# AnnaUshnova/tinyrenderder

Measured on AMD Instinct MI355X. Metric: triangles/sec (+ Mpixels/sec) at 4096x4096; achieved HBM GB/s vs peak, higher is better.
Workload: dtype f64

## Files before the change

tinyrenderder_amd/csrc/kernels_bin.hip:

```cpp
#include <hip/hip_runtime.h>
#include "trgl_device.h"
#include "launch.h"

namespace {

__device__ __forceinline__ double dmin3(double a, double b, double c) { double m = a; if (b < m) m = b; if (c < m) m = c; return m; }
__device__ __forceinline__ double dmax3(double a, double b, double c) { double m = a; if (m < b) m = b; if (m < c) m = c; return m; }
__device__ __forceinline__ double dot4(const double* m, const double* v) {
    double sum = 0;
    sum += m[0] * v[0]; sum += m[1] * v[1]; sum += m[2] * v[2]; sum += m[3] * v[3];
    return sum;
}

__device__ __forceinline__ int wave_min_i(int v) {
    for (int o = 32; o; o >>= 1) { int t = __shfl_xor(v, o); v = t < v ? t : v; }
    return v;
}
__device__ __forceinline__ int wave_max_i(int v) {
    for (int o = 32; o; o >>= 1) { int t = __shfl_xor(v, o); v = t > v ? t : v; }
    return v;
}

constexpr int SETUP_THREADS = 256;

__global__ __launch_bounds__(SETUP_THREADS) void k_setup(FrameParams fp, DrawDesc d, DrawDesc* __restrict__ draws_out, int draw_idx,
                                                         TriRec* __restrict__ recs, TriW* __restrict__ recs_w, uint32_t* __restrict__ cnt,
                                                         uint2* __restrict__ tilebox, DevStats* __restrict__ stats,
                                                         uint32_t* __restrict__ blk_sums, uint32_t blk_base) {
    __shared__ __attribute__((aligned(16))) double s_buf[SETUP_THREADS * 16];
    if (blockIdx.x == 0 && threadIdx.x == 0) draws_out[draw_idx] = d;
    const uint32_t b0 = blockIdx.x * SETUP_THREADS;
    const uint32_t nb = min((uint32_t)SETUP_THREADS, d.n - b0);
    const uint32_t tid = threadIdx.x;
    const uint32_t i = b0 + tid;
    const bool in_range = tid < nb;

    const double* src = d.clip + (size_t)b0 * 12;
    if ((reinterpret_cast<uintptr_t>(src) & 15) == 0) {
        const double2* s2 = reinterpret_cast<const double2*>(src);
        double2* l2 = reinterpret_cast<double2*>(s_buf);
        typedef double f64x2 __attribute__((ext_vector_type(2)));
        for (uint32_t k = tid; k < nb * 6; k += SETUP_THREADS)
            *reinterpret_cast<f64x2*>(&l2[k]) = __builtin_nontemporal_load(reinterpret_cast<const f64x2*>(&s2[k]));
    } else {
        for (uint32_t k = tid; k < nb * 12; k += SETUP_THREADS) s_buf[k] = src[k];
    }
    __syncthreads();
    double v[12];
#pragma unroll
    for (int k = 0; k < 12; ++k) v[k] = in_range ? s_buf[tid * 12 + k] : 0.0;
    __syncthreads();

    int bx0 = INT_MAX, by0 = INT_MAX, bx1 = INT_MIN, by1 = INT_MIN;
    uint32_t ntiles = 0;
    bool large = false;
    uint2 tb = make_uint2(0, 0);
    TriRec r;
    {
        uint4* z4 = reinterpret_cast<uint4*>(&r);
#pragma unroll
        for (int k = 0; k < 8; ++k) z4[k] = make_uint4(0, 0, 0, 0);
    }
    if (in_range) {
        bool ok = !(v[3] <= 1e-12 || v[7] <= 1e-12 || v[11] <= 1e-12);
        double ndc[12];
#pragma unroll
        for (int q = 0; q < 3; ++q) {
#pragma unroll
            for (int k = 0; k < 3; ++k) ndc[4 * q + k] = v[4 * q + k] / v[4 * q + 3];
            ndc[4 * q + 3] = __builtin_isfinite(v[4 * q + 3]) ? 1.0 : __builtin_nan("");
        }
        bool zo0 = (ndc[2] < -1.0 || ndc[2] > 1.0), zo1 = (ndc[6] < -1.0 || ndc[6] > 1.0),
             zo2 = (ndc[10] < -1.0 || ndc[10] > 1.0);
        ok = ok && !(zo0 && zo1 && zo2);
#pragma unroll
        for (int k = 0; k < 12; ++k) ok = ok && __builtin_isfinite(ndc[k]);
        double sx[3], sy[3];
#pragma unroll
        for (int q = 0; q < 3; ++q) { sx[q] = dot4(fp.vp, ndc + 4 * q); sy[q] = dot4(fp.vp + 4, ndc + 4 * q); }
        double e1x = sx[1] - sx[0], e1y = sy[1] - sy[0], e2x = sx[2] - sx[0], e2y = sy[2] - sy[0];
        double cross_product = e1x * e2y - e1y * e2x;
        ok = ok && !(cross_product <= 0);
        int min_x_px = max(0, x86_cvttsd2si(floor(dmin3(sx[0], sx[1], sx[2]))));
        int max_x_px = min(fp.W - 1, x86_cvttsd2si(ceil(dmax3(sx[0], sx[1], sx[2]))));
        int min_y_px = max(0, x86_cvttsd2si(floor(dmin3(sy[0], sy[1], sy[2]))));
        int max_y_px = min(fp.H - 1, x86_cvttsd2si(ceil(dmax3(sy[0], sy[1], sy[2]))));
        ok = ok && !(min_x_px > max_x_px || min_y_px > max_y_px);
        if (ok) {
            bx0 = min_x_px; by0 = min_y_px; bx1 = max_x_px; by1 = max_y_px;
            r.ax = sx[0]; r.ay = sy[0];
            r.s0x = sx[2] - sx[0]; r.s0y = sx[1] - sx[0];
            r.s1x = sy[2] - sy[0]; r.s1y = sy[1] - sy[0];
            r.uz = r.s0x * r.s1y - r.s0y * r.s1x;
            {
                const double BIG = 0x1p200, SMALL = 0x1p-250;
                bool ws = r.uz < 0.0 && !(fabs(r.uz) < 1e-12);
#pragma unroll
                for (int q = 0; q < 3; ++q) ws = ws && fabs(sx[q]) < BIG && fabs(sy[q]) < BIG;
                const double dl[4] = { r.s0x, r.s0y, r.s1x, r.s1y };
#pragma unroll
                for (int q = 0; q < 4; ++q) ws = ws && (dl[q] == 0.0 || fabs(dl[q]) >= SMALL);
                {
                    const double S = (fabs(r.s0x) + fabs(r.s0y)) + (fabs(r.s1x) + fabs(r.s1y));
                    const double rx = fmax(fabs(r.ax - ((double)bx0 + 0.5)), fabs(r.ax - ((double)bx1 + 0.5)));
                    const double ry = fmax(fabs(r.ay - ((double)by0 + 0.5)), fabs(r.ay - ((double)by1 + 0.5)));
                    ws = ws && 0x1p-40 * (S * S) * (rx + ry + 17.0 + S) < fabs(r.uz);
                }
                r.ruz = ws ? 1.0 / r.uz : 0.0;
            }
            r.z0 = ndc[2]; r.z1 = ndc[6]; r.z2 = ndc[10];
            r.bx0 = (uint16_t)bx0; r.by0 = (uint16_t)by0; r.bx1 = (uint16_t)bx1; r.by1 = (uint16_t)by1;
            r.color = d.colors ? d.colors[i] : 0xffffffffu;
            r.dl = ((uint32_t)draw_idx << 24) | i | (r.ruz == 0.0 ? TRGL_DL_LITERAL : 0u);
            r.c0 = -__builtin_inf(); r.g1 = 0.0; r.g2 = 0.0;
            if (r.ruz != 0.0) {
                const double zabs = dmax3(fabs(r.z0), fabs(r.z1), fabs(r.z2));
                const double dz1 = r.z1 - r.z0, dz2 = r.z2 - r.z0;
                const double h1 = (r.s1x * dz1 - r.s1y * dz2) * r.ruz, h2 = (r.s0y * dz2 - r.s0x * dz1) * r.ruz;
                const double rx = fmax(fabs(r.ax - ((double)bx0 + 0.5)), fabs(r.ax - ((double)bx1 + 0.5)));
                const double ry = fmax(fabs(r.ay - ((double)by0 + 0.5)), fabs(r.ay - ((double)by1 + 0.5)));
                const double Ssum = (fabs(r.s0x) + fabs(r.s0y)) + (fabs(r.s1x) + fabs(r.s1y));
                const double R = rx + ry + 1.0 + Ssum;
                const double mz = zabs * 0x1p-39 * (R * Ssum * fabs(r.ruz) + 1.0) + 0x1p-600;
                const bool okp = zabs < 0x1p1000 && R * fabs(h1) < 0x1p900 && R * fabs(h2) < 0x1p900 && mz < 0x1p1000;
                if (okp) { r.c0 = r.z0 - mz; r.g1 = h1; r.g2 = h2; }
            }
            if (d.kind != TRGL_SHADER_FLAT) {
                TriW w;
                w.iw0 = (fabs(v[3]) > 1e-12) ? (1.0 / v[3]) : 0.0;
                w.iw1 = (fabs(v[7]) > 1e-12) ? (1.0 / v[7]) : 0.0;
                w.iw2 = (fabs(v[11]) > 1e-12) ? (1.0 / v[11]) : 0.0;
                w.pad = 0.0;
                recs_w[d.first + i] = w;
            }
            int y_lo = max(by0, fp.strip_y0), y_hi = min(by1, fp.strip_y1 - 1);
            if (!(fabs(r.uz) < 1e-12) && y_lo <= y_hi) {
                uint32_t tx0 = bx0 >> TRGL_TILE_LOG2, tx1 = bx1 >> TRGL_TILE_LOG2;
                uint32_t ty0 = y_lo >> TRGL_TILE_LOG2, ty1 = y_hi >> TRGL_TILE_LOG2;
                const uint32_t rows = fp.il_tiles ? (uint32_t)(il_owned_below(fp, (int)ty1 + 1) - il_owned_below(fp, (int)ty0)) : ty1 - ty0 + 1;
                ntiles = (tx1 - tx0 + 1) * rows;
                tb = make_uint2(((uint32_t)bx0 >> TRGL_BLOCK_LOG2) | (((uint32_t)y_lo >> TRGL_BLOCK_LOG2) << 16),
                                ((uint32_t)bx1 >> TRGL_BLOCK_LOG2) | (((uint32_t)y_hi >> TRGL_BLOCK_LOG2) << 16));
                uint32_t zq = 0;
                if (r.c0 > -__builtin_inf()) {
                    const double zv = dmin3(r.c0, __builtin_fma(-r.s0y, r.g1, __builtin_fma(-r.s1y, r.g2, r.c0)),
                                            __builtin_fma(-r.s0x, r.g1, __builtin_fma(-r.s1x, r.g2, r.c0)));
                    const double t = (zv + 1.0) * 64.0 - 0x1p-20;
                    if (t >= 1.0) zq = t >= 127.0 ? 127u : (uint32_t)x86_cvttsd2si(floor(t));
                }
                tb.x |= (zq & 7u) << 13; tb.y |= ((zq >> 3) & 7u) << 13; tb.y |= (zq >> 6) << 29;
                large = bx1 - bx0 >= 64 || y_hi - y_lo >= 64;
            }
        }
        cnt[d.first + i] = ntiles;
        tilebox[d.first + i] = tb;
    }
    const uint32_t lane = tid & 63, wbase = tid & ~63u;
    {
        uint4* l4 = reinterpret_cast<uint4*>(s_buf);
        const uint4* r4 = reinterpret_cast<const uint4*>(&r);
#pragma unroll
        for (int c = 0; c < 8; ++c) l4[tid * 8 + (c ^ (tid & 7))] = r4[c];
        const unsigned long long keep = __ballot(ntiles != 0);
        __builtin_amdgcn_wave_barrier();
        uint4* dst = reinterpret_cast<uint4*>(recs + d.first + b0 + wbase);
#pragma unroll
        for (int it = 0; it < 8; ++it) {
            const uint32_t k = lane + 64u * it, t = k >> 3, c = k & 7;
            if ((keep >> t) & 1ull) {
                typedef uint32_t u32x4 __attribute__((ext_vector_type(4)));
                __builtin_nontemporal_store(*reinterpret_cast<const u32x4*>(&l4[(wbase + t) * 8 + (c ^ (t & 7))]), reinterpret_cast<u32x4*>(&dst[k]));
            }
        }
    }
    {
        uint32_t ws = ntiles;
        for (int o = 32; o; o >>= 1) ws += __shfl_xor(ws, o);
        __syncthreads();
        uint32_t* s_ws = reinterpret_cast<uint32_t*>(s_buf);
        if (lane == 0) s_ws[tid >> 6] = ws;
        __syncthreads();
        if (tid == 0) blk_sums[blk_base + blockIdx.x] = s_ws[0] + s_ws[1] + s_ws[2] + s_ws[3];
    }
    {
        const unsigned long long lit = __ballot(ntiles != 0 && r.ruz == 0.0);
        if (lit && lane == 0) atomicAdd(&stats->literal_tris, (unsigned long long)__popcll(lit));
        const unsigned long long lrg = __ballot(large);
        if (lrg && lane == 0) atomicAdd(&stats->large_tris, (unsigned long long)__popcll(lrg));
    }
    int wx0 = wave_min_i(bx0), wy0 = wave_min_i(by0), wx1 = wave_max_i(bx1), wy1 = wave_max_i(by1);
    if ((threadIdx.x & 63) == 0 && wx0 != INT_MAX) {
        if (wx0 < __builtin_nontemporal_load(&stats->min_x)) atomicMin(&stats->min_x, wx0);
        if (wy0 < __builtin_nontemporal_load(&stats->min_y)) atomicMin(&stats->min_y, wy0);
        if (wx1 > __builtin_nontemporal_load(&stats->max_x)) atomicMax(&stats->max_x, wx1);
        if (wy1 > __builtin_nontemporal_load(&stats->max_y)) atomicMax(&stats->max_y, wy1);
    }
}

constexpr int SCAN_THREADS = 256;

__device__ __forceinline__ uint32_t wave_incl_scan(uint32_t v) {
    int lane = threadIdx.x & 63;
    for (int o = 1; o < 64; o <<= 1) { uint32_t t = __shfl_up(v, o); if (lane >= o) v += t; }
    return v;
}

__device__ __forceinline__ uint32_t block_excl_scan(uint32_t v, uint32_t* smem , uint32_t* total) {
    uint32_t inc = wave_incl_scan(v);
    int w = threadIdx.x >> 6, lane = threadIdx.x & 63;
    __syncthreads();
    if (lane == 63) smem[w] = inc;
    __syncthreads();
    uint32_t base = 0, tot = 0;
#pragma unroll
    for (int k = 0; k < SCAN_THREADS / 64; ++k) { uint32_t s = smem[k]; if (k < w) base += s; tot += s; }
    *total = tot;
    return base + inc - v;
}

constexpr int EXPAND_CHUNK = 16;

constexpr int SPINE_THREADS = 1024;
__global__ __launch_bounds__(SPINE_THREADS) void k_chunk_spine(const uint32_t* __restrict__ blk_sums, uint32_t nblk,
                                                               uint32_t* __restrict__ chunk_off,
                                                               unsigned long long* __restrict__ total64, unsigned long long* __restrict__ host_copy,
                                                               uint4* __restrict__ bounds16, uint32_t n_half16) {
    __shared__ unsigned long long s_wave[SPINE_THREADS / 64];
    for (uint32_t k = threadIdx.x; k < 2 * n_half16; k += SPINE_THREADS) bounds16[k] = k < n_half16 ? make_uint4(~0u, ~0u, ~0u, ~0u) : make_uint4(0, 0, 0, 0);
    const uint32_t nchunks = (nblk + EXPAND_CHUNK - 1) / EXPAND_CHUNK;
    const int lane = threadIdx.x & 63, w = threadIdx.x >> 6;
    unsigned long long running = 0;
    for (uint32_t start = 0; start < nchunks; start += SPINE_THREADS) {
        const uint32_t c = start + threadIdx.x;
        unsigned long long v = 0;
        if (c < nchunks) {
            const uint32_t q0 = c * EXPAND_CHUNK;
            if (q0 + EXPAND_CHUNK <= nblk) {
                const uint4* p4 = reinterpret_cast<const uint4*>(blk_sums + q0);
#pragma unroll
                for (int k = 0; k < EXPAND_CHUNK / 4; ++k) { const uint4 t = p4[k]; v += (unsigned long long)t.x + t.y + t.z + t.w; }
            } else {
                for (uint32_t q = q0; q < nblk; ++q) v += blk_sums[q];
            }
        }
        unsigned long long inc = v;
        for (int o = 1; o < 64; o <<= 1) { const unsigned long long t = __shfl_up(inc, o); if (lane >= o) inc += t; }
        if (lane == 63) s_wave[w] = inc;
        __syncthreads();
        unsigned long long base = 0, tot = 0;
#pragma unroll
        for (int k = 0; k < SPINE_THREADS / 64; ++k) { const unsigned long long t = s_wave[k]; if (k < w) base += t; tot += t; }
        if (c < nchunks) chunk_off[c] = (uint32_t)(running + base + inc - v);
        running += tot;
        __syncthreads();
    }
    if (threadIdx.x == 0) {
        *total64 = running;
        host_copy[0] = running; host_copy[1] = total64[1]; host_copy[2] = total64[2];
        __threadfence_system();
    }
}

constexpr uint32_t EXPAND_STAGE = 3072;
__device__ __forceinline__ uint32_t tile_block_mask(uint32_t tx, uint32_t ty, uint32_t qx0, uint32_t qy0, uint32_t qx1, uint32_t qy1) {
    const uint32_t c0 = qx0 > 4 * tx ? qx0 - 4 * tx : 0u, c1 = qx1 < 4 * tx + 3 ? qx1 - 4 * tx : 3u;
    const uint32_t r0 = qy0 > 4 * ty ? qy0 - 4 * ty : 0u, r1 = qy1 < 4 * ty + 3 ? qy1 - 4 * ty : 3u;
    return (((2u << c1) - (1u << c0)) & 0xfu) * 0x1111u & ((0xffffu >> (12 - 4 * r1)) & (0xffffu << (4 * r0)));
}
template <bool WIDE>
__global__ __launch_bounds__(256) void k_expand(FrameParams fp, uint32_t first, uint32_t n, int tiles_x, const uint32_t* __restrict__ cnt,
                                                const uint32_t* __restrict__ blk_sums, const uint32_t* __restrict__ chunk_off,
                                                uint32_t blk_base, const uint2* __restrict__ tilebox,
                                                uint32_t* __restrict__ keys, uint32_t* __restrict__ vals, uint16_t* __restrict__ bmask,
                                                const unsigned long long* __restrict__ pairs_total, uint32_t cap) {
    __shared__ uint32_t smem[4];
    __shared__ __attribute__((aligned(16))) uint32_t s_k[EXPAND_STAGE + 4];
    __shared__ __attribute__((aligned(16))) uint32_t s_v[EXPAND_STAGE + 4];
    __shared__ __attribute__((aligned(16))) uint16_t s_m[WIDE ? EXPAND_STAGE + 4 : 4];
    if (*pairs_total > cap) return;
    const uint32_t local = blockIdx.x * blockDim.x + threadIdx.x;
    const uint32_t i = first + local;
    const uint32_t blk = blk_base + blockIdx.x;
    uint32_t c = 0; uint2 tb = make_uint2(0, 0);
    if (local < n) { c = cnt[i]; if (c) tb = tilebox[i]; }
    uint32_t base;
    {
        const uint32_t q0 = blk - blk % EXPAND_CHUNK, l = threadIdx.x & 63u;
        uint32_t part = l < blk - q0 ? blk_sums[q0 + l] : 0u;
        for (int o = 8; o; o >>= 1) part += __shfl_xor(part, o);
        base = chunk_off[blk / EXPAND_CHUNK] + (uint32_t)__builtin_amdgcn_readfirstlane((int)part);
    }
    uint32_t tot;
    const uint32_t o = block_excl_scan(c, smem, &tot);
    const bool staged = tot <= EXPAND_STAGE;
    const uint32_t sh = base & 3u;
    uint32_t* const kdst = keys + base; uint32_t* const vdst = vals + base; uint16_t* const mdst = bmask + base;
    auto put = [&](uint32_t j, uint32_t key, uint32_t iz, uint32_t m) {
        const uint32_t word = WIDE ? key : key | (m << 16);
        if (staged) { s_k[sh + j] = word; s_v[sh + j] = iz; if (WIDE) s_m[sh + j] = (uint16_t)m; }
        else { kdst[j] = word; vdst[j] = iz; if (WIDE) mdst[j] = (uint16_t)m; }
    };
    constexpr uint32_t SMALL = 8;
    if (c && c <= SMALL) {
        const uint32_t qx0 = tb.x & 0x1fff, qy0 = (tb.x >> 16) & 0x1fff, qx1 = tb.y & 0x1fff, qy1 = (tb.y >> 16) & 0x1fff;
        const uint32_t iz = i | ((((tb.x >> 13) & 7u) | (((tb.y >> 13) & 7u) << 3) | ((tb.y >> 29) << 6)) << 25);
        const uint32_t tx0 = qx0 >> 2, ty0 = qy0 >> 2, tx1 = qx1 >> 2;
        uint32_t tx = tx0, row = 0;
        uint32_t ty = fp.il_tiles ? (uint32_t)il_nth_owned_from(fp, (int)ty0, 0) : ty0;
        for (uint32_t k = 0; k < c; ++k) {
            put(o + k, ty * tiles_x + tx, iz, tile_block_mask(tx, ty, qx0, qy0, qx1, qy1));
            if (++tx > tx1) { tx = tx0; ++row; ty = fp.il_tiles ? (uint32_t)il_nth_owned_from(fp, (int)ty0, (int)row) : ty0 + row; }
        }
    }
    unsigned long long big = __ballot(c > SMALL);
    int lane = threadIdx.x & 63;
    while (big) {
        int src = __ffsll((long long)big) - 1;
        big &= big - 1;
        uint32_t cc = __shfl(c, src), oo = __shfl(o, src), ii = __shfl(i, src);
        uint32_t bx = __shfl(tb.x, src), by = __shfl(tb.y, src);
        const uint32_t qx0 = bx & 0x1fff, qy0 = (bx >> 16) & 0x1fff, qx1 = by & 0x1fff, qy1 = (by >> 16) & 0x1fff;
        ii |= (((bx >> 13) & 7u) | (((by >> 13) & 7u) << 3) | ((by >> 29) << 6)) << 25;
        uint32_t tx0 = qx0 >> 2, ty0 = qy0 >> 2, tx1 = qx1 >> 2;
        uint32_t wdt = tx1 - tx0 + 1;
        for (uint32_t k = lane; k < cc; k += 64) {
            uint32_t ty = fp.il_tiles ? (uint32_t)il_nth_owned_from(fp, (int)ty0, (int)(k / wdt)) : ty0 + k / wdt, tx = tx0 + k % wdt;
            put(oo + k, ty * tiles_x + tx, ii, tile_block_mask(tx, ty, qx0, qy0, qx1, qy1));
        }
    }
    if (staged) {
        __syncthreads();
        uint32_t* const kq = keys + (base - sh); uint32_t* const vq = vals + (base - sh); uint16_t* const mq = bmask + (base - sh);
        const uint32_t end = sh + tot;
        for (uint32_t q = threadIdx.x; 4 * q < end; q += 256) {
            const uint32_t j0 = 4 * q;
            if (j0 >= sh && j0 + 4 <= end) {
                *reinterpret_cast<uint4*>(kq + j0) = *reinterpret_cast<const uint4*>(s_k + j0);
                *reinterpret_cast<uint4*>(vq + j0) = *reinterpret_cast<const uint4*>(s_v + j0);
                if (WIDE) *reinterpret_cast<uint2*>(mq + j0) = *reinterpret_cast<const uint2*>(s_m + j0);
            } else {
                for (uint32_t j = j0; j < j0 + 4; ++j)
                    if (j >= sh && j < end) { kq[j] = s_k[j]; vq[j] = s_v[j]; if (WIDE) mq[j] = s_m[j]; }
            }
        }
    }
}

constexpr int RADIX_ROUNDS = 16;
constexpr int RADIX_WAVE_CHUNK = RADIX_ROUNDS * 64;
constexpr uint32_t RADIX_BIG_CAP = 4u << 20;
constexpr int RADIX_MAX_BITS = 8;

__global__ __launch_bounds__(256) void k_radix_hist(const uint32_t* __restrict__ keys, const unsigned long long* __restrict__ pairs_total,
                                                    uint32_t cap, int shift, int bits, uint32_t chunk,
                                                    uint32_t nblocks, uint32_t* __restrict__ hist) {
    __shared__ uint32_t s_cnt[1 << RADIX_MAX_BITS];
    const unsigned long long P64 = *pairs_total;
    const uint32_t P = P64 > cap ? 0u : (uint32_t)P64;
    const uint32_t nb = 1u << bits, mask = nb - 1;
    for (uint32_t b = threadIdx.x; b < nb; b += 256) s_cnt[b] = 0;
    __syncthreads();
    const uint64_t beg = (uint64_t)blockIdx.x * chunk;
    uint64_t end = beg + chunk; if (end > P) end = P;
    for (uint64_t p = beg + 4u * threadIdx.x; p < end; p += 1024) {
        const uint4 q = *reinterpret_cast<const uint4*>(keys + p);
        const uint32_t k[4] = { q.x, q.y, q.z, q.w };
#pragma unroll
        for (int j = 0; j < 4; ++j) if (p + j < end) atomicAdd(&s_cnt[(k[j] >> shift) & mask], 1u);
    }
    __syncthreads();
    for (uint32_t b = threadIdx.x; b < nb; b += 256) hist[(size_t)b * nblocks + blockIdx.x] = s_cnt[b];
}

constexpr int ROWSCAN_THREADS = 1024, ROWSCAN_PER = 8;
__global__ __launch_bounds__(ROWSCAN_THREADS) void k_radix_scan_rows(uint32_t* __restrict__ hist, uint32_t nblocks, uint32_t* __restrict__ totals) {
    __shared__ uint32_t s_wave[ROWSCAN_THREADS / 64];
    uint32_t* row = hist + (size_t)blockIdx.x * nblocks;
    const int lane = threadIdx.x & 63, w = threadIdx.x >> 6;
    uint32_t running = 0;
    for (uint32_t start = 0; start < nblocks; start += ROWSCAN_THREADS * ROWSCAN_PER) {
        const uint32_t base = start + threadIdx.x * ROWSCAN_PER;
        uint32_t v[ROWSCAN_PER], sum = 0;
#pragma unroll
        for (int k = 0; k < ROWSCAN_PER; ++k) { v[k] = (base + k < nblocks) ? row[base + k] : 0; sum += v[k]; }
        uint32_t inc = sum;
        for (int o = 1; o < 64; o <<= 1) { const uint32_t t = __shfl_up(inc, o); if (lane >= o) inc += t; }
        if (lane == 63) s_wave[w] = inc;
        __syncthreads();
        uint32_t wbase = 0, tot = 0;
#pragma unroll
        for (int k = 0; k < ROWSCAN_THREADS / 64; ++k) { const uint32_t t = s_wave[k]; if (k < w) wbase += t; tot += t; }
        uint32_t run = running + wbase + inc - sum;
#pragma unroll
        for (int k = 0; k < ROWSCAN_PER; ++k) { if (base + k < nblocks) row[base + k] = run; run += v[k]; }
        running += tot;
        __syncthreads();
    }
    if (threadIdx.x == 0) totals[blockIdx.x] = running;
}

template <int RADIX_WAVES, bool WIDE, bool LAST>
__global__ __launch_bounds__(RADIX_WAVES * 64) void k_radix_scatter(const uint32_t* __restrict__ keys_in, const uint32_t* __restrict__ vals_in,
                                                                 const uint16_t* __restrict__ msk_in,
                                                                 const unsigned long long* __restrict__ pairs_total, uint32_t cap,
                                                                 int shift, int bits, uint32_t nblocks,
                                                                 const uint32_t* __restrict__ base, const uint32_t* __restrict__ totals,
                                                                 uint32_t* __restrict__ keys_out, uint32_t* __restrict__ vals_out,
                                                                 uint16_t* __restrict__ msk_out,
                                                                 uint32_t* __restrict__ tile_start, uint32_t* __restrict__ tile_end) {
    constexpr int RADIX_THREADS = RADIX_WAVES * 64, RADIX_CHUNK = RADIX_WAVES * RADIX_WAVE_CHUNK;
    __shared__ uint32_t s_cnt[RADIX_WAVES][1 << RADIX_MAX_BITS];
    __shared__ uint32_t s_start[1 << RADIX_MAX_BITS];
    __shared__ uint32_t s_gbase[1 << RADIX_MAX_BITS];
    __shared__ uint32_t s_val[RADIX_CHUNK];
    __shared__ uint32_t s_key[RADIX_CHUNK];
    __shared__ uint16_t s_msk[WIDE ? RADIX_CHUNK : 2];
    const int w = threadIdx.x >> 6, lane = threadIdx.x & 63;
    const unsigned long long P64 = *pairs_total;
    const uint32_t P = P64 > cap ? 0u : (uint32_t)P64;
    if ((uint64_t)blockIdx.x * RADIX_CHUNK >= P) return;
    const uint32_t nb = 1u << bits, mask = nb - 1;
    for (uint32_t b = threadIdx.x; b < nb; b += RADIX_THREADS) {
#pragma unroll
        for (int ww = 0; ww < RADIX_WAVES; ++ww) s_cnt[ww][b] = 0;
        s_gbase[b] = base[(size_t)b * nblocks + blockIdx.x];
    }
    if (w == 0) {
        uint32_t tot[4], run = 0;
#pragma unroll
        for (int q = 0; q < 4; ++q) { const uint32_t d = lane * 4 + q; tot[q] = d < nb ? totals[d] : 0; run += tot[q]; }
        uint32_t inc = run;
        for (int o = 1; o < 64; o <<= 1) { const uint32_t t = __shfl_up(inc, o); if (lane >= o) inc += t; }
        uint32_t ex = inc - run;
#pragma unroll
        for (int q = 0; q < 4; ++q) { const uint32_t d = lane * 4 + q; if (d < nb) s_start[d] = ex; ex += tot[q]; }
    }
    __syncthreads();
    for (uint32_t b = threadIdx.x; b < nb; b += RADIX_THREADS) s_gbase[b] += s_start[b];
    __syncthreads();
    const uint64_t cbeg = (uint64_t)blockIdx.x * RADIX_CHUNK;
    uint64_t cend = cbeg + RADIX_CHUNK; if (cend > P) cend = P;
    const uint32_t n_chunk = (uint32_t)(cend - cbeg);
    const uint64_t wbeg = cbeg + (uint64_t)w * RADIX_WAVE_CHUNK;
    const unsigned long long lt = (1ull << lane) - 1ull;

    uint32_t k[RADIX_ROUNDS], v[RADIX_ROUNDS], rk[RADIX_ROUNDS];
    uint16_t mk[WIDE ? RADIX_ROUNDS : 1];
#pragma unroll
    for (int r = 0; r < RADIX_ROUNDS; ++r) {
        const uint64_t p = wbeg + (uint64_t)r * 64 + lane;
        const bool act = p < cend;
        k[r] = act ? keys_in[p] : 0; v[r] = act ? vals_in[p] : 0;
        if (WIDE) mk[WIDE ? r : 0] = act ? msk_in[p] : (uint16_t)0;
    }
#pragma unroll
    for (int r = 0; r < RADIX_ROUNDS; ++r) {
        const bool act = wbeg + (uint64_t)r * 64 + lane < cend;
        const uint32_t dgt = (k[r] >> shift) & mask;
        unsigned long long same = __ballot(act);
        for (int b = 0; b < bits; ++b) {
            const unsigned long long bal = __ballot((dgt >> b) & 1u);
            same &= ((dgt >> b) & 1u) ? bal : ~bal;
        }
        const uint32_t cur = act ? s_cnt[w][dgt] : 0;
        __builtin_amdgcn_wave_barrier();
        const uint32_t r_in = __popcll(same & lt);
        rk[r] = cur + r_in;
        if (act && r_in == 0) s_cnt[w][dgt] = cur + (uint32_t)__popcll(same);
        __builtin_amdgcn_wave_barrier();
    }
    __syncthreads();
    if (w == 0) {
        uint32_t tot[4], run = 0;
#pragma unroll
        for (int q = 0; q < 4; ++q) {
            const uint32_t d = lane * 4 + q;
            uint32_t t = 0;
            if (d < nb) {
#pragma unroll
                for (int ww = 0; ww < RADIX_WAVES; ++ww) t += s_cnt[ww][d];
            }
            tot[q] = t;
            run += tot[q];
        }
        uint32_t inc = run;
        for (int o = 1; o < 64; o <<= 1) { const uint32_t t = __shfl_up(inc, o); if (lane >= o) inc += t; }
        uint32_t ex = inc - run;
#pragma unroll
        for (int q = 0; q < 4; ++q) { const uint32_t d = lane * 4 + q; if (d < nb) s_start[d] = ex; ex += tot[q]; }
    }
    __syncthreads();
    for (uint32_t d = threadIdx.x; d < nb; d += RADIX_THREADS) {
        uint32_t run = s_start[d];
#pragma unroll
        for (int ww = 0; ww < RADIX_WAVES; ++ww) { const uint32_t c = s_cnt[ww][d]; s_cnt[ww][d] = run; run += c; }
    }
    __syncthreads();
#pragma unroll
    for (int r = 0; r < RADIX_ROUNDS; ++r) {
        if (wbeg + (uint64_t)r * 64 + lane < cend) {
            const uint32_t dgt = (k[r] >> shift) & mask;
            const uint32_t lp = s_cnt[w][dgt] + rk[r];
            s_key[lp] = k[r]; s_val[lp] = v[r];
            if (WIDE) s_msk[lp] = mk[WIDE ? r : 0];
        }
    }
    __syncthreads();
    constexpr uint32_t KEY_MASK = WIDE ? 0xffffffffu : 0xffffu;
    for (uint32_t i = threadIdx.x; i < n_chunk; i += RADIX_THREADS) {
        const uint32_t word = s_key[i];
        const uint32_t dgt = (word >> shift) & mask;
        const uint32_t dst = s_gbase[dgt] + (i - s_start[dgt]);
        vals_out[dst] = s_val[i];
        if (!LAST) {
            keys_out[dst] = word;
            if (WIDE) msk_out[dst] = s_msk[i];
        } else {
            msk_out[dst] = WIDE ? s_msk[i] : (uint16_t)(word >> 16);
            const uint32_t key = word & KEY_MASK;
            if (i == 0 || (s_key[i - 1] & KEY_MASK) != key) atomicMin(&tile_start[key], dst);
            if (i + 1 == n_chunk || (s_key[i + 1] & KEY_MASK) != key) atomicMax(&tile_end[key], dst + 1);
        }
    }
}

}

namespace trgl {

uint32_t setup_num_blocks(uint32_t n) { return (n + SETUP_THREADS - 1) / SETUP_THREADS; }

void launch_setup(hipStream_t s, const FrameParams& fp, const DrawDesc& draw, DrawDesc* draws_dev, int draw_idx, uint32_t n,
                  TriRec* recs, TriW* recs_w, uint32_t* cnt, uint2* tilebox, DevStats* stats, uint32_t* blk_sums, uint32_t blk_base) {
    if (!n) return;
    hipLaunchKernelGGL(k_setup, dim3(setup_num_blocks(n)), dim3(SETUP_THREADS), 0, s, fp, draw, draws_dev, draw_idx, recs, recs_w, cnt, tilebox,
                       stats, blk_sums, blk_base);
}

void launch_chunk_spine(hipStream_t s, const uint32_t* blk_sums, uint32_t nblk, uint32_t* chunk_off, unsigned long long* total64, unsigned long long* host_copy,
                        uint32_t* tile_bounds, size_t half_words) {
    hipLaunchKernelGGL(k_chunk_spine, dim3(1), dim3(SPINE_THREADS), 0, s, blk_sums, nblk, chunk_off, total64, host_copy, (uint4*)tile_bounds,
                       (uint32_t)(half_words / 4));
}

void launch_expand(hipStream_t s, const FrameParams& fp, uint32_t first, uint32_t n, int tiles_x, const uint32_t* cnt, const uint32_t* blk_sums,
                   const uint32_t* chunk_off, uint32_t blk_base, const uint2* tilebox, uint32_t* keys, bool wide, uint32_t* vals, uint16_t* bmask,
                   const unsigned long long* pairs_total, uint32_t cap) {
    if (!n) return;
    if (wide)
        hipLaunchKernelGGL(k_expand<true>, dim3(setup_num_blocks(n)), dim3(SETUP_THREADS), 0, s, fp, first, n, tiles_x, cnt, blk_sums, chunk_off,
                           blk_base, tilebox, keys, vals, bmask, pairs_total, cap);
    else
        hipLaunchKernelGGL(k_expand<false>, dim3(setup_num_blocks(n)), dim3(SETUP_THREADS), 0, s, fp, first, n, tiles_x, cnt, blk_sums, chunk_off,
                           blk_base, tilebox, keys, vals, bmask, pairs_total, cap);
}

static uint32_t radix_waves(uint32_t cap) { return cap >= RADIX_BIG_CAP ? 8u : 4u; }
uint32_t radix_num_workers(uint32_t cap) { const uint64_t chunk = radix_waves(cap) * RADIX_WAVE_CHUNK; return (uint32_t)((cap + chunk - 1) / chunk); }

template <int WAVES, bool WIDE, bool LAST>
static void radix_pass_t(hipStream_t s, const RadixPass& ps, const unsigned long long* pairs_total, uint32_t cap, uint32_t* hist, uint32_t* scan_tmp) {
    const uint32_t nblk = radix_num_workers(cap);
    hipLaunchKernelGGL(k_radix_hist, dim3(nblk), dim3(256), 0, s, ps.keys_in, pairs_total, cap, ps.shift, ps.bits, (uint32_t)(WAVES * RADIX_WAVE_CHUNK),
                       nblk, hist);
    hipLaunchKernelGGL(k_radix_scan_rows, dim3(1u << ps.bits), dim3(ROWSCAN_THREADS), 0, s, hist, nblk, scan_tmp);
    hipLaunchKernelGGL((k_radix_scatter<WAVES, WIDE, LAST>), dim3(nblk), dim3(WAVES * 64), 0, s, ps.keys_in, ps.vals_in, ps.msk_in, pairs_total, cap,
                       ps.shift, ps.bits, nblk, hist, scan_tmp, ps.keys_out, ps.vals_out, ps.msk_out, ps.tile_start, ps.tile_end);
}

template <int WAVES>
static void radix_pass_w(hipStream_t s, const RadixPass& ps, bool wide, bool last, const unsigned long long* pairs_total, uint32_t cap,
                         uint32_t* hist, uint32_t* scan_tmp) {
    if (wide) { if (last) radix_pass_t<WAVES, true, true>(s, ps, pairs_total, cap, hist, scan_tmp); else radix_pass_t<WAVES, true, false>(s, ps, pairs_total, cap, hist, scan_tmp); }
    else { if (last) radix_pass_t<WAVES, false, true>(s, ps, pairs_total, cap, hist, scan_tmp); else radix_pass_t<WAVES, false, false>(s, ps, pairs_total, cap, hist, scan_tmp); }
}

void launch_radix_pass(hipStream_t s, const RadixPass& ps, bool wide, bool last, const unsigned long long* pairs_total, uint32_t cap,
                       uint32_t* hist, uint32_t* scan_tmp) {
    if (!cap) return;
    if (radix_waves(cap) == 8) radix_pass_w<8>(s, ps, wide, last, pairs_total, cap, hist, scan_tmp);
    else radix_pass_w<4>(s, ps, wide, last, pairs_total, cap, hist, scan_tmp);
}

}
```

Before: 4.120 billion.

## Hoist global loads ahead of dependent work in expand and radix kernels

In the expand kernel, the per-block prefix loads (blk_sums, chunk_off, tilebox) are issued before the early-exit check so their latency overlaps. The radix histogram is templated on a fixed step count and issues all of its uint4 key loads up front, clamping the tail address, before doing the shared atomics. The scatter kernel issues the bucket-base and totals loads together with the key/value loads and moves its shared init and scan after them. Its output phase is batched into groups of eight so shared reads and address math are done before the global stores. The cost targeted is serialized memory latency, in exchange for more registers per thread and heavier unrolling, which may lower occupancy.

```diff
diff --git a/tinyrenderder_amd/csrc/kernels_bin.hip b/tinyrenderder_amd/csrc/kernels_bin.hip
--- a/tinyrenderder_amd/csrc/kernels_bin.hip
+++ b/tinyrenderder_amd/csrc/kernels_bin.hip
@@ -277,18 +277,19 @@
     __shared__ __attribute__((aligned(16))) uint32_t s_k[EXPAND_STAGE + 4];
     __shared__ __attribute__((aligned(16))) uint32_t s_v[EXPAND_STAGE + 4];
     __shared__ __attribute__((aligned(16))) uint16_t s_m[WIDE ? EXPAND_STAGE + 4 : 4];
-    if (*pairs_total > cap) return;
     const uint32_t local = blockIdx.x * blockDim.x + threadIdx.x;
     const uint32_t i = first + local;
     const uint32_t blk = blk_base + blockIdx.x;
     uint32_t c = 0; uint2 tb = make_uint2(0, 0);
-    if (local < n) { c = cnt[i]; if (c) tb = tilebox[i]; }
+    if (local < n) { c = cnt[i]; tb = tilebox[i]; }
+    const uint32_t q0 = blk - blk % EXPAND_CHUNK, l = threadIdx.x & 63u;
+    uint32_t part = l < blk - q0 ? blk_sums[q0 + l] : 0u;
+    const uint32_t coff = chunk_off[blk / EXPAND_CHUNK];
+    if (*pairs_total > cap) return;
     uint32_t base;
     {
-        const uint32_t q0 = blk - blk % EXPAND_CHUNK, l = threadIdx.x & 63u;
-        uint32_t part = l < blk - q0 ? blk_sums[q0 + l] : 0u;
         for (int o = 8; o; o >>= 1) part += __shfl_xor(part, o);
-        base = chunk_off[blk / EXPAND_CHUNK] + (uint32_t)__builtin_amdgcn_readfirstlane((int)part);
+        base = coff + (uint32_t)__builtin_amdgcn_readfirstlane((int)part);
     }
     uint32_t tot;
     const uint32_t o = block_excl_scan(c, smem, &tot);
@@ -351,9 +352,10 @@
 constexpr uint32_t RADIX_BIG_CAP = 4u << 20;
 constexpr int RADIX_MAX_BITS = 8;
 
+template <int STEPS>
 __global__ __launch_bounds__(256) void k_radix_hist(const uint32_t* __restrict__ keys, const unsigned long long* __restrict__ pairs_total,
-                                                    uint32_t cap, int shift, int bits, uint32_t chunk,
-                                                    uint32_t nblocks, uint32_t* __restrict__ hist) {
+                                                    uint32_t cap, int shift, int bits, uint32_t nblocks, uint32_t* __restrict__ hist) {
+    constexpr uint32_t chunk = STEPS * 1024;
     __shared__ uint32_t s_cnt[1 << RADIX_MAX_BITS];
     const unsigned long long P64 = *pairs_total;
     const uint32_t P = P64 > cap ? 0u : (uint32_t)P64;
@@ -362,9 +364,18 @@
     __syncthreads();
     const uint64_t beg = (uint64_t)blockIdx.x * chunk;
     uint64_t end = beg + chunk; if (end > P) end = P;
-    for (uint64_t p = beg + 4u * threadIdx.x; p < end; p += 1024) {
-        const uint4 q = *reinterpret_cast<const uint4*>(keys + p);
-        const uint32_t k[4] = { q.x, q.y, q.z, q.w };
+    if (beg >= end) { for (uint32_t b = threadIdx.x; b < nb; b += 256) hist[(size_t)b * nblocks + blockIdx.x] = 0; return; }
+    const uint64_t last4 = (end - 1) & ~(uint64_t)3;
+    uint4 q[STEPS];
+#pragma unroll
+    for (int r = 0; r < STEPS; ++r) {
+        const uint64_t p = beg + 4u * threadIdx.x + 1024u * r;
+        q[r] = *reinterpret_cast<const uint4*>(keys + (p < last4 ? p : last4));
+    }
+#pragma unroll
+    for (int r = 0; r < STEPS; ++r) {
+        const uint64_t p = beg + 4u * threadIdx.x + 1024u * r;
+        const uint32_t k[4] = { q[r].x, q[r].y, q[r].z, q[r].w };
 #pragma unroll
         for (int j = 0; j < 4; ++j) if (p + j < end) atomicAdd(&s_cnt[(k[j] >> shift) & mask], 1u);
     }
@@ -409,6 +420,7 @@
                                                                  uint16_t* __restrict__ msk_out,
                                                                  uint32_t* __restrict__ tile_start, uint32_t* __restrict__ tile_end) {
     constexpr int RADIX_THREADS = RADIX_WAVES * 64, RADIX_CHUNK = RADIX_WAVES * RADIX_WAVE_CHUNK;
+    static_assert(RADIX_THREADS >= (1 << RADIX_MAX_BITS), "one thread per digit");
     __shared__ uint32_t s_cnt[RADIX_WAVES][1 << RADIX_MAX_BITS];
     __shared__ uint32_t s_start[1 << RADIX_MAX_BITS];
     __shared__ uint32_t s_gbase[1 << RADIX_MAX_BITS];
@@ -420,30 +432,17 @@
     const uint32_t P = P64 > cap ? 0u : (uint32_t)P64;
     if ((uint64_t)blockIdx.x * RADIX_CHUNK >= P) return;
     const uint32_t nb = 1u << bits, mask = nb - 1;
-    for (uint32_t b = threadIdx.x; b < nb; b += RADIX_THREADS) {
-#pragma unroll
-        for (int ww = 0; ww < RADIX_WAVES; ++ww) s_cnt[ww][b] = 0;
-        s_gbase[b] = base[(size_t)b * nblocks + blockIdx.x];
-    }
-    if (w == 0) {
-        uint32_t tot[4], run = 0;
-#pragma unroll
-        for (int q = 0; q < 4; ++q) { const uint32_t d = lane * 4 + q; tot[q] = d < nb ? totals[d] : 0; run += tot[q]; }
-        uint32_t inc = run;
-        for (int o = 1; o < 64; o <<= 1) { const uint32_t t = __shfl_up(inc, o); if (lane >= o) inc += t; }
-        uint32_t ex = inc - run;
-#pragma unroll
-        for (int q = 0; q < 4; ++q) { const uint32_t d = lane * 4 + q; if (d < nb) s_start[d] = ex; ex += tot[q]; }
-    }
-    __syncthreads();
-    for (uint32_t b = threadIdx.x; b < nb; b += RADIX_THREADS) s_gbase[b] += s_start[b];
-    __syncthreads();
     const uint64_t cbeg = (uint64_t)blockIdx.x * RADIX_CHUNK;
     uint64_t cend = cbeg + RADIX_CHUNK; if (cend > P) cend = P;
     const uint32_t n_chunk = (uint32_t)(cend - cbeg);
     const uint64_t wbeg = cbeg + (uint64_t)w * RADIX_WAVE_CHUNK;
     const unsigned long long lt = (1ull << lane) - 1ull;
 
+    const uint32_t dq = min((uint32_t)threadIdx.x, nb - 1);
+    const uint32_t gcol = base[(size_t)dq * nblocks + blockIdx.x];
+    uint32_t tot[4];
+#pragma unroll
+    for (int q = 0; q < 4; ++q) { const uint32_t d = lane * 4 + q; tot[q] = totals[min(d, nb - 1)]; if (d >= nb) tot[q] = 0; }
     uint32_t k[RADIX_ROUNDS], v[RADIX_ROUNDS], rk[RADIX_ROUNDS];
     uint16_t mk[WIDE ? RADIX_ROUNDS : 1];
 #pragma unroll
@@ -453,6 +452,24 @@
         k[r] = act ? keys_in[p] : 0; v[r] = act ? vals_in[p] : 0;
         if (WIDE) mk[WIDE ? r : 0] = act ? msk_in[p] : (uint16_t)0;
     }
+    if (threadIdx.x < nb) {
+#pragma unroll
+        for (int ww = 0; ww < RADIX_WAVES; ++ww) s_cnt[ww][threadIdx.x] = 0;
+        s_gbase[threadIdx.x] = gcol;
+    }
+    if (w == 0) {
+        uint32_t run = 0;
+#pragma unroll
+        for (int q = 0; q < 4; ++q) run += tot[q];
+        uint32_t inc = run;
+        for (int o = 1; o < 64; o <<= 1) { const uint32_t t = __shfl_up(inc, o); if (lane >= o) inc += t; }
+        uint32_t ex = inc - run;
+#pragma unroll
+        for (int q = 0; q < 4; ++q) { const uint32_t d = lane * 4 + q; if (d < nb) s_start[d] = ex; ex += tot[q]; }
+    }
+    __syncthreads();
+    if (threadIdx.x < nb) s_gbase[threadIdx.x] += s_start[threadIdx.x];
+
 #pragma unroll
     for (int r = 0; r < RADIX_ROUNDS; ++r) {
         const bool act = wbeg + (uint64_t)r * 64 + lane < cend;
@@ -490,8 +507,10 @@
         for (int q = 0; q < 4; ++q) { const uint32_t d = lane * 4 + q; if (d < nb) s_start[d] = ex; ex += tot[q]; }
     }
     __syncthreads();
-    for (uint32_t d = threadIdx.x; d < nb; d += RADIX_THREADS) {
+    if (threadIdx.x < nb) {
+        const uint32_t d = threadIdx.x;
         uint32_t run = s_start[d];
+        s_gbase[d] -= run;
 #pragma unroll
         for (int ww = 0; ww < RADIX_WAVES; ++ww) { const uint32_t c = s_cnt[ww][d]; s_cnt[ww][d] = run; run += c; }
     }
@@ -507,19 +526,39 @@
     }
     __syncthreads();
     constexpr uint32_t KEY_MASK = WIDE ? 0xffffffffu : 0xffffu;
-    for (uint32_t i = threadIdx.x; i < n_chunk; i += RADIX_THREADS) {
-        const uint32_t word = s_key[i];
-        const uint32_t dgt = (word >> shift) & mask;
-        const uint32_t dst = s_gbase[dgt] + (i - s_start[dgt]);
-        vals_out[dst] = s_val[i];
-        if (!LAST) {
-            keys_out[dst] = word;
-            if (WIDE) msk_out[dst] = s_msk[i];
-        } else {
-            msk_out[dst] = WIDE ? s_msk[i] : (uint16_t)(word >> 16);
-            const uint32_t key = word & KEY_MASK;
-            if (i == 0 || (s_key[i - 1] & KEY_MASK) != key) atomicMin(&tile_start[key], dst);
-            if (i + 1 == n_chunk || (s_key[i + 1] & KEY_MASK) != key) atomicMax(&tile_end[key], dst + 1);
+    constexpr int OUT_STEPS = RADIX_CHUNK / RADIX_THREADS, OUT_BATCH = 8;
+    static_assert(OUT_STEPS % OUT_BATCH == 0, "phase 4 batches");
+#pragma unroll
+    for (int r0 = 0; r0 < OUT_STEPS; r0 += OUT_BATCH) {
+        uint32_t word[OUT_BATCH], val[OUT_BATCH], dst[OUT_BATCH], prev[LAST ? OUT_BATCH : 1], next[LAST ? OUT_BATCH : 1];
+        uint16_t m[WIDE ? OUT_BATCH : 1];
+#pragma unroll
+        for (int j = 0; j < OUT_BATCH; ++j) {
+            const uint32_t i = threadIdx.x + (uint32_t)(r0 + j) * RADIX_THREADS;
+            word[j] = s_key[i]; val[j] = s_val[i];
+            if (WIDE) m[WIDE ? j : 0] = s_msk[i];
+            if (LAST) { prev[LAST ? j : 0] = s_key[i ? i - 1 : 0]; next[LAST ? j : 0] = s_key[min(i + 1, (uint32_t)RADIX_CHUNK - 1)]; }
+        }
+#pragma unroll
+        for (int j = 0; j < OUT_BATCH; ++j) {
+            const uint32_t i = threadIdx.x + (uint32_t)(r0 + j) * RADIX_THREADS;
+            dst[j] = s_gbase[(word[j] >> shift) & mask] + i;
+        }
+#pragma unroll
+        for (int j = 0; j < OUT_BATCH; ++j) {
+            const uint32_t i = threadIdx.x + (uint32_t)(r0 + j) * RADIX_THREADS;
+            if (i < n_chunk) {
+                vals_out[dst[j]] = val[j];
+                if (!LAST) {
+                    keys_out[dst[j]] = word[j];
+                    if (WIDE) msk_out[dst[j]] = m[WIDE ? j : 0];
+                } else {
+                    msk_out[dst[j]] = WIDE ? m[WIDE ? j : 0] : (uint16_t)(word[j] >> 16);
+                    const uint32_t key = word[j] & KEY_MASK;
+                    if (i == 0 || (prev[LAST ? j : 0] & KEY_MASK) != key) atomicMin(&tile_start[key], dst[j]);
+                    if (i + 1 == n_chunk || (next[LAST ? j : 0] & KEY_MASK) != key) atomicMax(&tile_end[key], dst[j] + 1);
+                }
+            }
         }
     }
 }
@@ -561,8 +600,8 @@
 template <int WAVES, bool WIDE, bool LAST>
 static void radix_pass_t(hipStream_t s, const RadixPass& ps, const unsigned long long* pairs_total, uint32_t cap, uint32_t* hist, uint32_t* scan_tmp) {
     const uint32_t nblk = radix_num_workers(cap);
-    hipLaunchKernelGGL(k_radix_hist, dim3(nblk), dim3(256), 0, s, ps.keys_in, pairs_total, cap, ps.shift, ps.bits, (uint32_t)(WAVES * RADIX_WAVE_CHUNK),
-                       nblk, hist);
+    static_assert(RADIX_WAVE_CHUNK == 1024, "a k_radix_hist step is 256 threads x 4 pairs");
+    hipLaunchKernelGGL(k_radix_hist<WAVES>, dim3(nblk), dim3(256), 0, s, ps.keys_in, pairs_total, cap, ps.shift, ps.bits, nblk, hist);
     hipLaunchKernelGGL(k_radix_scan_rows, dim3(1u << ps.bits), dim3(ROWSCAN_THREADS), 0, s, hist, nblk, scan_tmp);
     hipLaunchKernelGGL((k_radix_scatter<WAVES, WIDE, LAST>), dim3(nblk), dim3(WAVES * 64), 0, s, ps.keys_in, ps.vals_in, ps.msk_in, pairs_total, cap,
                        ps.shift, ps.bits, nblk, hist, scan_tmp, ps.keys_out, ps.vals_out, ps.msk_out, ps.tile_start, ps.tile_end);
```

Result: no change. 4.160 billion, median of 6 (+1.0%).
